# lucashilbig/BA_Pathtracing_Fur

Hardware: AMD Instinct MI355X
Metric: Msamples/s at 1080p 8spp, 1M-strand hairball; achieved HBM GB/s vs peak (higher is better)
Workload: dtype f32

## Files before the change

ba_pathtracing_fur_amd/csrc/render.hip:

```cpp
#include <hip/hip_runtime.h>
#include <rccl/rccl.h>
#include <stdio.h>
#include <string.h>

#include <algorithm>
#include <chrono>
#include <memory>
#include <string>
#include <condition_variable>
#include <deque>
#include <mutex>
#include <thread>
#include <type_traits>
#include <vector>

#include "device.h"
#include "device_build.h"
#include "lightpath.h"

using namespace khp;

#ifndef KHP_MAX_SEG
#define KHP_MAX_SEG 64
#endif
// ... 155 lines not shown
    c->nqb[0] = 0;
}

__global__ void k_prep(Counters* c, ShadowQ* q, int cur) {
    int nxt = cur ^ 1;
    c->nq[nxt] = 0;
    c->nqb[nxt] = 0;
    q->nsh = 0;
    q->nshb = 0;
    for (int g = 0; g < KHP_MAX_SEG; ++g) {
        c->fetch_ext[32 * g] = 0;
        q->fetch[32 * g] = 0;
    }
    c->ext_rays += c->nq[cur] + c->nqb[cur];
}

#ifndef KHP_EXT_RING
#define KHP_EXT_RING 8
#endif
#ifndef KHP_EXT_WAVES
#define KHP_EXT_WAVES 6
#endif
#ifndef KHP_EXT_REFILL
#define KHP_EXT_REFILL 24
#endif
#ifndef KHP_SH_RING
#define KHP_SH_RING 8
#endif
#ifndef KHP_SH_WAVES
#define KHP_SH_WAVES 6
#endif
constexpr int RING = KHP_SH_RING;
constexpr int REFILL = 24;
constexpr int TRAV_WAVES = KHP_SH_WAVES;
constexpr int EXT_RING = KHP_EXT_RING;
constexpr int EXT_WAVES = KHP_EXT_WAVES;
#ifndef KHP_EXT_WAVES_W
#define KHP_EXT_WAVES_W 6
#endif
constexpr int EXT_WAVES_W = KHP_EXT_WAVES_W;
#ifndef KHP_REFILL_CAM
#define KHP_REFILL_CAM 28
#endif
#ifndef KHP_REFILL_NARROW
#define KHP_REFILL_NARROW 28
#endif
#ifndef KHP_REFILL_WIDE
#define KHP_REFILL_WIDE 16
#endif
constexpr size_t LDS_BYTES = 3 * RING * TRAV_BLOCK * sizeof(uint32_t);
constexpr size_t EXT_LDS_BYTES = 3 * EXT_RING * TRAV_BLOCK * sizeof(uint32_t);
#ifndef KHP_CAM_RING
#define KHP_CAM_RING 6
#endif
#ifndef KHP_CAM_WAVES
#define KHP_CAM_WAVES 8
#endif
constexpr int CAM_RING = KHP_CAM_RING;
constexpr int CAM_WAVES = KHP_CAM_WAVES;
constexpr size_t CAM_LDS_BYTES = 3 * CAM_RING * TRAV_BLOCK * sizeof(uint32_t);
template <bool STATS, bool TOP = false>
using TravStack = LdsStack<RING, STATS, TOP>;
template <bool STATS, bool CAM = false, bool TOP = false>
using ExtStack = LdsStack<CAM ? CAM_RING : EXT_RING, STATS, TOP>;
constexpr size_t TOP_LDS_BYTES = TOP_NODES * sizeof(DevNode);

// ... 114 lines not shown
}

__device__ __forceinline__ void mark_pixel(const Wave& Wv, uint32_t pid, bool long_ray) {
    uint32_t fr, p_local, s_local;
    path_coords(Wv, pid, fr, p_local, s_local);
    Wv.pixheavy[Wv.pix[Wv.p_off + p_local]] = long_ray ? 1 : 0;
}

__global__ __launch_bounds__(256) void k_pix_order(const uint32_t* __restrict__ pix, uint32_t n,
                                                  const uint8_t* __restrict__ heavy, uint32_t* __restrict__ out,
                                                  uint32_t* cnt) {
    const uint32_t i = blockIdx.x * blockDim.x + threadIdx.x;
    const bool in = i < n;
    const uint32_t px = in ? pix[i] : 0u;
    const bool hv = in && heavy[px] != 0;
    const uint32_t f = wave_alloc(hv, &cnt[0]);
    const uint32_t b = wave_alloc(in && !hv, &cnt[1]);
    if (hv) out[f] = px;
    else if (in) out[n - 1u - b] = px;
}

template <bool STATS, bool CAM = false, bool WIDE = false, bool TOP = false>
__global__ __launch_bounds__(TRAV_BLOCK, WIDE ? EXT_WAVES_W : CAM ? CAM_WAVES : EXT_WAVES) void k_extend(DevScene S, Wave Wv, int cur, SpillArea spill) {
    extern __shared__ uint32_t lds[];
    const uint32_t nf = Wv.cnt->nq[cur], nb = Wv.cnt->nqb[cur];
    ExtStack<STATS, CAM, TOP> stk;
    stk.init(lds, spill.base, spill.stride);
    if (TOP) stk.stage_top(S.top);
    TravStats st{0, 0, 0};
    TravRay tr;
    Hit h;
    Cur c{0u, 0.0f, 0.0f, false};
    LeafCur lf{0u, 0u, 0.0f, 0.0f, 0.0f, 0.0f, -1};
    bool has = false, exhausted = false;
    uint32_t idx = 0, mode = 0u;
    unsigned long long wit = 0, wbusy = 0;
    uint32_t it = 0;
    Claimer cl;
    cl.init(Wv.cnt->fetch_ext, nf, nb, Wv.cap);
    constexpr int refill = WIDE ? KHP_REFILL_WIDE : CAM ? KHP_REFILL_CAM : KHP_REFILL_NARROW;
    for (;;) {
        unsigned long long idle = __ballot(!has);
        if (!exhausted && __popcll(idle) >= refill) {
            uint32_t my;
            const bool got = cl.claim(idle, my, exhausted);
            if (!has && got && cl.phys(my, idx)) {
                it = 0;
                Ray r;
                if (CAM) {
                    uint32_t key_unused;
                    r = camera_path(S, Wv, idx, key_unused);
                } else {
                    r.o = mk(Wv.qo[cur][0][idx], Wv.qo[cur][1][idx], Wv.qo[cur][2][idx]);
                    r.d = mk(Wv.qd[cur][0][idx], Wv.qd[cur][1][idx], Wv.qd[cur][2][idx]);
                }
                trav_setup(tr, r);
                h.t = FLT_MAX_;
                h.slot = -1;
                h.u = h.v = 0.0f;
                lf.left = 0;
                has = (STATS || !ray_has_nan(r)) && trav2_begin<STATS>(S, tr, h.t, stk, mode, c, lf, st);
                if (!has) {
                    Wv.ht[idx] = h.t;
                    Wv.hslot[idx] = -1;
                    Wv.heavy[idx] = 0;
                    if (CAM && Wv.pixheavy) mark_pixel(Wv, idx, false);
                }
            }
        }
        unsigned long long act = __ballot(has);
        if (act == 0) {
            if (exhausted) break;
            continue;
        }
        for (;;) {
            if (STATS) {
                unsigned long long wm = __ballot(has && (mode == M_NODE || mode == M_LEAF));
                ++wit;
                wbusy += (uint32_t)__popcll(wm);
            }
            if (has) {
                bool occ_unused;
                ++it;
                const bool fin = WIDE ? iterw<false, STATS>(S, tr, h, 0.0f, stk, mode, c, lf, st, occ_unused)
                                      : iter2<false, STATS>(S, tr, h, 0.0f, stk, mode, c, lf, st, occ_unused);
                if (fin) {
                    uint32_t j = idx;
                    asm volatile("" : "+v"(j));
                    Wv.ht[j] = h.t;
                    Wv.hslot[j] = h.slot;
                    Wv.heavy[j] = it > Wv.heavy_T ? 1 : 0;
                    if (CAM && Wv.pixheavy) mark_pixel(Wv, j, it > Wv.heavy_T);
                    has = false;
                }
            }
            act = __ballot(has);
            if (act == 0 || (!exhausted && 64 - __popcll(act) >= refill)) break;
        }
    }
    if (STATS)
        flush_stats(st, stk, wit, wbusy, &Wv.cnt->node_visits, &Wv.cnt->prim_tests, &Wv.cnt->pruned, &Wv.cnt->iters,
                    &Wv.cnt->lanes_busy, &Wv.cnt->spills);
}

static void launch_extend(bool stats, bool cam, bool wide, int grid, hipStream_t s, const DevScene& S, const Wave& W,
                          int cur, SpillArea sp, bool top = false) {
    const dim3 g(grid), b(TRAV_BLOCK);
    if (top && !stats && !wide && S.top) {
        if (cam) hipLaunchKernelGGL((k_extend<false, true, false, true>), g, b, CAM_LDS_BYTES + TOP_LDS_BYTES, s, S, W, cur, sp);
        else hipLaunchKernelGGL((k_extend<false, false, false, true>), g, b, EXT_LDS_BYTES + TOP_LDS_BYTES, s, S, W, cur, sp);
        return;
    }
#define KHP_EXT(ST, CA, WI) \
    hipLaunchKernelGGL((k_extend<ST, CA, WI>), g, b, CA ? CAM_LDS_BYTES : EXT_LDS_BYTES, s, S, W, cur, sp)
    if (wide) {
        if (stats) { if (cam) KHP_EXT(true, true, true); else KHP_EXT(true, false, true); }
        else { if (cam) KHP_EXT(false, true, true); else KHP_EXT(false, false, true); }
    } else {
        if (stats) { if (cam) KHP_EXT(true, true, false); else KHP_EXT(true, false, false); }
        else { if (cam) KHP_EXT(false, true, false); else KHP_EXT(false, false, false); }
    }
#undef KHP_EXT
}

__device__ __forceinline__ void textured_material(const DevScene& S, const Aux& ax, const float4* pr, v3 loc,
                                               const ShadeCtx& s, float bu, float bv, khp_material& out);
template <bool TEX>
__device__ __forceinline__ v3 surface_at(const DevScene& S, const Ray& r, const Hit& h, ShadeCtx& s,
                                         khp_material& mres) {
// ... 713 lines not shown
        const float4 f = rec[5];
        acc = acc + mk(f.x, f.y, f.z);
    }
    (void)pid;
    float4* dst = state_dest(Wv, nxt, bits_from_f(e.w));
    const float4 ck = *dst;
    *dst = make_float4(ck.x + acc.x, ck.y + acc.y, ck.z + acc.z, ck.w);
}

template <bool BD>
__global__ __launch_bounds__(256) void k_shadow_finish(DevScene S, Wave Wv, int nxt) {
    const uint32_t nf = Wv.shq->nsh, n = nf + Wv.shq->nshb;
    if (blockIdx.x == 0 && threadIdx.x == 0) atomicAdd(&Wv.cnt->sh_rays, (unsigned long long)n);
    for (uint32_t iv = blockIdx.x * blockDim.x + threadIdx.x; iv < n; iv += gridDim.x * blockDim.x) {
        const uint32_t i = q_phys(iv, nf, Wv.cap);
        if (BD) connection_group_finish(S, Wv, nxt, i);
        else shadow_finish_one(S, Wv, nxt, i, Wv.vis[i] != 0);
    }
}

template <bool STATS, bool WIDE = false, bool TOP = false>
__global__ __launch_bounds__(TRAV_BLOCK, TRAV_WAVES) void k_shadow(DevScene S, Wave Wv, SpillArea spill) {
    extern __shared__ uint32_t lds[];
    const uint32_t nf = Wv.shq->nsh, nb = Wv.shq->nshb;
    TravStack<STATS, TOP> stk;
    stk.init(lds, spill.base, spill.stride);
    if (TOP) stk.stage_top(S.top);
    TravStats st{0, 0, 0};
    TravRay tr;
    Cur c{0u, 0.0f, 0.0f, false};
    LeafCur lf{0u, 0u, 0.0f, 0.0f, 0.0f, 0.0f, -1};
    unsigned long long wit = 0, wbusy = 0;
    float tmax = 0.0f;
    uint32_t mode = 0u;
    bool has = false, exhausted = false;
    Claimer cl;
    cl.init(Wv.shq->fetch, nf, nb, Wv.cap);
    uint32_t idx = 0;
    for (;;) {
        unsigned long long idle = __ballot(!has);
        if (!exhausted && __popcll(idle) >= REFILL) {
            uint32_t my;
            const bool got = cl.claim(idle, my, exhausted);
            if (!has && got && cl.phys(my, idx)) {
                const float4* rec = Wv.sh + Wv.shs * (size_t)idx;
                float4 a = rec[0], b = rec[1];
                Ray r;
                r.o = mk(a.x, a.y, a.z);
                r.d = mk(b.x, b.y, b.z);
                tmax = a.w;
                trav_setup(tr, r);
                lf.left = 0;
                if (!STATS && x_slab_nan(tr)) {
                    has = false;
                    Wv.vis[idx] = any_hit_x_nan(S, r) ? 1 : 0;
                } else {
                    has = trav2_begin<STATS>(S, tr, tmax, stk, mode, c, lf, st);
                    if (!has) Wv.vis[idx] = 0;
                }
            }
        }
        unsigned long long act = __ballot(has);
        if (act == 0) {
            if (exhausted) break;
            continue;
        }
        for (;;) {
            if (STATS) {
                unsigned long long wm = __ballot(has && (mode == M_NODE || mode == M_LEAF));
                ++wit;
                wbusy += (uint32_t)__popcll(wm);
            }
            if (has) {
                bool occ = false;
                Hit hu_{0.0f, -1, 0.0f, 0.0f};
                const bool fin = WIDE ? iterw<true, STATS>(S, tr, hu_, tmax, stk, mode, c, lf, st, occ)
                                      : iter2<true, STATS>(S, tr, hu_, tmax, stk, mode, c, lf, st, occ);
                if (fin) {
                    Wv.vis[idx] = occ ? 1 : 0;
                    has = false;
                }
            }
            act = __ballot(has);
            if (act == 0 || (!exhausted && 64 - __popcll(act) >= REFILL)) break;
        }
    }
    if (STATS)
        flush_stats(st, stk, wit, wbusy, &Wv.cnt->sh_node_visits, &Wv.cnt->sh_prim_tests, &Wv.cnt->sh_pruned,
                    &Wv.cnt->sh_iters, &Wv.cnt->sh_lanes_busy, &Wv.cnt->spills);
}

static void launch_shadow(bool stats, bool wide, int grid, hipStream_t s, const DevScene& S, const Wave& W, SpillArea sp,
                          bool top = false) {
    const dim3 g(grid), b(TRAV_BLOCK);
    if (top && !stats && !wide && S.top) {
        hipLaunchKernelGGL((k_shadow<false, false, true>), g, b, LDS_BYTES + TOP_LDS_BYTES, s, S, W, sp);
        return;
    }
    if (wide) {
        if (stats) hipLaunchKernelGGL((k_shadow<true, true>), g, b, LDS_BYTES, s, S, W, sp);
        else hipLaunchKernelGGL((k_shadow<false, true>), g, b, LDS_BYTES, s, S, W, sp);
    } else {
        if (stats) hipLaunchKernelGGL((k_shadow<true, false>), g, b, LDS_BYTES, s, S, W, sp);
        else hipLaunchKernelGGL((k_shadow<false, false>), g, b, LDS_BYTES, s, S, W, sp);
    }
}

#ifndef KHP_PATH_WAVES
#define KHP_PATH_WAVES 4
#endif
#ifndef KHP_PATH_RING
#define KHP_PATH_RING 8
#endif
#ifndef KHP_PATH_REFILL
#define KHP_PATH_REFILL 24
#endif
// ... 3156 lines not shown
        Wv.shq->nsh = as_shadow ? n : 0u;
    }
    if (i >= n) return;
    Ray r = make_ray(ld3(orig + 3 * (size_t)i), ld3(dir + 3 * (size_t)i));
    if (as_shadow) {
        Wv.sh[Wv.shs * (size_t)i] = make_float4(r.o.x, r.o.y, r.o.z, tmax[i]);
        Wv.sh[Wv.shs * (size_t)i + 1] = make_float4(r.d.x, r.d.y, r.d.z, 0.0f);
    } else {
        Wv.qo[0][0][i] = r.o.x; Wv.qo[0][1][i] = r.o.y; Wv.qo[0][2][i] = r.o.z;
        Wv.qd[0][0][i] = r.d.x; Wv.qd[0][1][i] = r.d.y; Wv.qd[0][2][i] = r.d.z;
    }
}

__global__ void k_store_hits(DevScene S, uint32_t n, Wave Wv, float* t, int32_t* obj, float* uv) {
    uint32_t i = blockIdx.x * blockDim.x + threadIdx.x;
    if (i >= n) return;
    int32_t sl = Wv.hslot[i];
    t[i] = Wv.ht[i];
    obj[i] = sl >= 0 ? (int32_t)S.aux[sl].obj : -1;
    float u = 0.0f, v = 0.0f;
    if (sl >= 0) {
        const float4* p = S.prims + 4 * (size_t)sl;
        if (is_tri(p[0])) {
            Ray r;
            r.o = mk(Wv.qo[0][0][i], Wv.qo[0][1][i], Wv.qo[0][2][i]);
            r.d = mk(Wv.qd[0][0][i], Wv.qd[0][1][i], Wv.qd[0][2][i]);
            tri_uv(p[0], p[1], p[2], r, u, v);
        }
    }
    uv[2 * i] = u;
    uv[2 * i + 1] = v;
}

static int trace_persistent(const khp_ctx* c) { return (int)c->prm.trace_kernels; }

static khp_status trace_persistent_run(khp_ctx* c, uint32_t n, const float* orig, const float* dir,
                                       const float* tmax_h, float* t_out, int32_t* obj_out, float* uv_out,
                                       uint8_t* hit_out) {
    const bool shadow = hit_out != nullptr;
    PathSet& w = c->ps[0];
    c->wa.valid = false;
    khp_status s = ensure_wave(c, w, n);
    if (s != KHP_OK) return s;
    DevMem o, d, tm, t, ob, uv;
    HIPCHK(upload(o, orig, 3 * (size_t)n, c->stream));
    HIPCHK(upload(d, dir, 3 * (size_t)n, c->stream));
    if (shadow) HIPCHK(upload(tm, tmax_h, (size_t)n, c->stream));
    HIPCHK(hipMemsetAsync(w.cnt.p, 0, sizeof(Counters), c->stream));
    HIPCHK(hipMemsetAsync(w.shqb.p, 0, 2 * sizeof(ShadowQ), c->stream));
    Wave Wv = wave_view(c, w);
    hipLaunchKernelGGL(k_load_rays, dim3((n + 255) / 256), dim3(256), 0, c->stream, n, o.as<float>(), d.as<float>(),
                       Wv, shadow ? 1 : 0, tm.as<float>());
    const bool prod = trace_persistent(c) == 2;
    hipEvent_t e0 = next_event(c), e1 = next_event(c);
    (void)hipEventRecord(e0, c->stream);
    if (shadow) {
        SpillArea sp{w.spill_sh.as<int4>(), (uint32_t)c->grid_sh * TRAV_BLOCK};
        const bool wide = c->S.wide != nullptr && c->prm.wide_from == 0;
        launch_shadow(!prod, wide, wide ? c->grid_sh_w : c->grid_sh, c->stream, c->S, Wv, sp);
        (void)hipEventRecord(e1, c->stream);
        HIPCHK(hipGetLastError());
        HIPCHK(hipMemcpyAsync(hit_out, Wv.vis, n, hipMemcpyDeviceToHost, c->stream));
    } else {
        SpillArea sp{w.spill.as<int4>(), (uint32_t)c->grid_ext_max * TRAV_BLOCK};
        const bool wide = c->S.wide != nullptr && c->prm.wide_from == 0;
        launch_extend(!prod, false, wide, wide ? c->grid_ext_w : c->grid_ext, c->stream, c->S, Wv, 0, sp);
        (void)hipEventRecord(e1, c->stream);
        HIPCHK(t.ensure(4 * (size_t)n));
        HIPCHK(ob.ensure(4 * (size_t)n));
        HIPCHK(uv.ensure(8 * (size_t)n));
        hipLaunchKernelGGL(k_store_hits, dim3((n + 255) / 256), dim3(256), 0, c->stream, c->S, n, Wv, t.as<float>(),
                           ob.as<int32_t>(), uv.as<float>());
        HIPCHK(hipGetLastError());
        HIPCHK(hipMemcpyAsync(t_out, t.p, 4 * (size_t)n, hipMemcpyDeviceToHost, c->stream));
        HIPCHK(hipMemcpyAsync(obj_out, ob.p, 4 * (size_t)n, hipMemcpyDeviceToHost, c->stream));
        if (uv_out) HIPCHK(hipMemcpyAsync(uv_out, uv.p, 8 * (size_t)n, hipMemcpyDeviceToHost, c->stream));
    }
    Counters hc;
    HIPCHK(hipMemcpyAsync(&hc, w.cnt.p, sizeof(hc), hipMemcpyDeviceToHost, c->stream));
    KHPCHK(wait_stream(c, c->stream, "the ray queries"));
    c->st.node_visits = shadow ? hc.sh_node_visits : hc.node_visits;
    c->st.prim_tests = shadow ? hc.sh_prim_tests : hc.prim_tests;
    c->st.stack_spills = hc.spills;
    float kms = 0.0f;
    (void)hipEventElapsedTime(&kms, e0, e1);
    c->st.render_ms = kms;
    c->ev_next = 0;
    return KHP_OK;
}

extern "C" khp_status khp_trace_closest(khp_ctx* c, uint32_t n, const float* orig, const float* dir, float* t_out,
                                        int32_t* obj_out, float* uv_out) {
    if (c) {
        khp_status dr = drain(c);
        if (dr != KHP_OK) return dr;
    }
    if (!c || (n && (!orig || !dir || !t_out || !obj_out))) return fail(KHP_EINVAL, "null argument");
    if (!c->built) return fail(KHP_ENOTREADY, "khp_build_accel first");
    if (n == 0) return KHP_OK;
    HIPCHK(hipSetDevice(c->device));
    if (trace_persistent(c)) return trace_persistent_run(c, n, orig, dir, nullptr, t_out, obj_out, uv_out, nullptr);
    DevMem o, d, t, ob, uv, stb;
    HIPCHK(upload(o, orig, 3 * (size_t)n, c->stream));
    HIPCHK(upload(d, dir, 3 * (size_t)n, c->stream));
    HIPCHK(t.ensure(4 * (size_t)n));
    HIPCHK(ob.ensure(4 * (size_t)n));
    HIPCHK(uv.ensure(8 * (size_t)n));
    HIPCHK(stb.ensure(16));
    HIPCHK(hipMemsetAsync(stb.p, 0, 16, c->stream));
    hipLaunchKernelGGL(k_trace_closest<true>, dim3((n + 255) / 256), dim3(256), 0, c->stream, c->S, n,
                       o.as<float>(), d.as<float>(), t.as<float>(), ob.as<int32_t>(), uv.as<float>(),
                       stb.as<unsigned long long>());
    HIPCHK(hipGetLastError());
    HIPCHK(hipMemcpyAsync(t_out, t.p, 4 * (size_t)n, hipMemcpyDeviceToHost, c->stream));
    HIPCHK(hipMemcpyAsync(obj_out, ob.p, 4 * (size_t)n, hipMemcpyDeviceToHost, c->stream));
    if (uv_out) HIPCHK(hipMemcpyAsync(uv_out, uv.p, 8 * (size_t)n, hipMemcpyDeviceToHost, c->stream));
// ... 443 lines not shown
```

ba_pathtracing_fur_amd/csrc/traverse.h:

```cpp
#pragma once

struct Hit {
    float t;
    int32_t slot;
    float u, v;
};

struct TravStats {
    uint32_t nodes, prims, pruned;
};

struct TravRay {
    Ray r;
    v3 inv;
    bool fin;
};

__device__ __forceinline__ void trav_setup(TravRay& tr, const Ray& r) {
    tr.r = r;
    tr.inv = mk(1.0f / r.d.x, 1.0f / r.d.y, 1.0f / r.d.z);
    tr.fin = __builtin_isfinite(tr.inv.x) && __builtin_isfinite(tr.inv.y) && __builtin_isfinite(tr.inv.z) &&
             __builtin_isfinite(r.o.x) && __builtin_isfinite(r.o.y) && __builtin_isfinite(r.o.z);
}

__device__ __forceinline__ bool ray_has_nan(const Ray& r) {
    return r.o.x != r.o.x || r.o.y != r.o.y || r.o.z != r.o.z || r.d.x != r.d.x || r.d.y != r.d.y ||
           r.d.z != r.d.z;
}

__device__ __forceinline__ bool x_slab_nan(const TravRay& tr) { return tr.inv.x != tr.inv.x || tr.r.o.x != tr.r.o.x; }
__device__ __forceinline__ bool any_hit_x_nan(const DevScene& S, const Ray& r) {
    for (uint32_t k = 0; k < S.n_tris; ++k) {
        const float4* p = S.prims + 4 * (size_t)S.tri_slot[k];
        const float4 ab = p[1], ac = p[2];
        const v3 dv = cross(r.d, mk(ac.x, ac.y, ac.z));
        const float det = dot(dv, mk(ab.x, ab.y, ab.z));
        if (!(fabsf(det) < TRI_EPS_D)) return true;
    }
    return false;
}

__device__ __forceinline__ bool ref_leaf(uint32_t r) { return (r & LEAF_BIT) != 0u; }

struct PrivStack {
    uint32_t ref[STACK_MAX];
    float t0[STACK_MAX], t1[STACK_MAX];
    int sp;
    __device__ __forceinline__ void clear() { sp = 0; }
    __device__ __forceinline__ bool empty() const { return sp == 0; }
    __device__ __forceinline__ void push(uint32_t r, float a, float b) {
        ref[sp] = r;
        t0[sp] = a;
        t1[sp] = b;
        ++sp;
    }
    __device__ __forceinline__ void pop(uint32_t& r, float& a, float& b) {
        --sp;
        r = ref[sp];
        a = t0[sp];
        b = t1[sp];
    }
};

#ifndef KHP_TRAV_BLOCK
#define KHP_TRAV_BLOCK 64
#endif
constexpr uint32_t TRAV_BLOCK = KHP_TRAV_BLOCK;

constexpr uint32_t TOP_NODES = 7;
constexpr uint32_t TOP_REF = 0x40000000u;
template <int R, bool COUNT, bool TOP = false>
struct LdsStack {
    static_assert(R >= 2 && R <= 16, "ring size");
    static constexpr bool kTop = TOP;
    static constexpr size_t kRingBytes = 3 * (size_t)R * TRAV_BLOCK * sizeof(uint32_t);
// ... 21 lines not shown
    __device__ __forceinline__ bool empty() const { return sp == 0; }
    __device__ __forceinline__ uint32_t slot(int e) const { return (uint32_t)((uint32_t)e % (uint32_t)R) * TRAV_BLOCK + threadIdx.x; }
    __device__ __forceinline__ int4* gcell(int e) const {
        return spill + (size_t)e * stride + blockIdx.x * blockDim.x + threadIdx.x;
    }
    __device__ __forceinline__ void push(uint32_t r, float a, float b) {
        if (sp - lo == R) {
            uint32_t k = slot(lo);
            *gcell(lo) = make_int4((int)lds[k], (int)lds[k + R * TRAV_BLOCK], (int)lds[k + 2 * R * TRAV_BLOCK], 0);
            ++lo;
            if (COUNT) ++spills;
        }
        uint32_t k = slot(sp);
        lds[k] = r;
        lds[k + R * TRAV_BLOCK] = bits_from_f(a);
        lds[k + 2 * R * TRAV_BLOCK] = bits_from_f(b);
        ++sp;
    }
    __device__ __forceinline__ void pop(uint32_t& r, float& a, float& b) {
        --sp;
        const uint32_t k = slot(sp);
        r = lds[k];
        a = f_from_bits(lds[k + R * TRAV_BLOCK]);
        b = f_from_bits(lds[k + 2 * R * TRAV_BLOCK]);
        asm volatile("" : "+v"(r), "+v"(a), "+v"(b));
        if (sp < lo) {
            int4 e = *gcell(sp);
            r = (uint32_t)e.x;
            a = f_from_bits((uint32_t)e.y);
            b = f_from_bits((uint32_t)e.z);
            lo = sp;
        }
    }
};

__device__ __forceinline__ void pin(float4& v) { asm volatile("" : "+v"(v.x), "+v"(v.y), "+v"(v.z), "+v"(v.w)); }
__device__ __forceinline__ void pin(int4& v) { asm volatile("" : "+v"(v.x), "+v"(v.y), "+v"(v.z), "+v"(v.w)); }

struct Cur {
    uint32_t ref;
    float t0, t1;
    bool valid;
};

template <class Stack>
__device__ __forceinline__ void cur_next(Stack& stk, Cur& c) {
    if (stk.empty()) {
        c.valid = false;
    } else {
        stk.pop(c.ref, c.t0, c.t1);
        c.valid = true;
    }
}


template <class Stack>
__device__ __forceinline__ bool trav_begin(const DevScene& S, const TravRay& tr, Stack& stk, Cur& c) {
    stk.clear();
    float t0, t1;
    c.valid = slab(S.root_box[0], S.root_box[1], S.root_box[2], S.root_box[3], S.root_box[4], S.root_box[5], tr.r,
                   tr.inv, t0, t1);
    c.ref = (uint32_t)S.root_ref;
    c.t0 = t0;
    c.t1 = t1;
    return c.valid;
}
// ... 152 lines not shown
    t0 = (tzmin > tmin) ? tzmin : tmin;
    t1 = (tzmax < tmax) ? tzmax : tmax;
    return ok;
}

__device__ __forceinline__ bool slab_fast(float mnx, float mny, float mnz, float mxx, float mxy, float mxz,
                                          const TravRay& tr, float& t0, float& t1) {
    const float ax = (mnx - tr.r.o.x) * tr.inv.x, bx = (mxx - tr.r.o.x) * tr.inv.x;
    const float ay = (mny - tr.r.o.y) * tr.inv.y, by = (mxy - tr.r.o.y) * tr.inv.y;
    const float az = (mnz - tr.r.o.z) * tr.inv.z, bz = (mxz - tr.r.o.z) * tr.inv.z;
    t0 = fmaxf(fmaxf(fminf(ax, bx), fminf(ay, by)), fminf(az, bz));
    t1 = fminf(fminf(fmaxf(ax, bx), fmaxf(ay, by)), fmaxf(az, bz));
    return t0 <= t1;
}

template <bool STATS>
__device__ __forceinline__ void take_entry(const DevScene& S, uint32_t ref, float t0, float t1, uint32_t& mode, Cur& c,
                                           LeafCur& lf, TravStats& st) {
    const bool leaf = ref_leaf(ref);
    c.ref = ref;
    c.t0 = t0;
    c.t1 = t1;
    mode = leaf ? M_LEAF : M_NODE;
    uint32_t cnt = (ref >> 24) & 0x7Fu;
    if (leaf && cnt == LEAF_CNT_ESC) cnt = S.aux[ref & 0x00FFFFFFu].flags >> 8;
    lf.slot = leaf ? (ref & 0x00FFFFFFu) : lf.slot;
    lf.left = leaf ? cnt : 0u;
    lf.tmax = t1;
    lf.tl = FLT_MAX_;
    lf.lu = 0.0f;
    lf.lv = 0.0f;
    lf.sl = -1;
    if (STATS && leaf) st.nodes++;
}

template <bool STATS, class Stack>
__device__ __forceinline__ bool trav2_begin(const DevScene& S, const TravRay& tr, float tlimit, Stack& stk,
                                            uint32_t& mode, Cur& c, LeafCur& lf, TravStats& st) {
    stk.clear();
    float t0, t1;
    if (!slab(S.root_box[0], S.root_box[1], S.root_box[2], S.root_box[3], S.root_box[4], S.root_box[5], tr.r,
              tr.inv, t0, t1))
        return false;
    if (t1 < 0.0f || t0 > tlimit) {
        if (STATS) st.pruned++;
        mode = M_POP;
        return true;
    }
    take_entry<STATS>(S, (uint32_t)(Stack::kTop ? S.top_root : S.root_ref), t0, t1, mode, c, lf, st);
    return true;
}

__device__ __forceinline__ bool candidate_rt(float4 p0, float4 p1, float4 p2, float4 p3, const Ray& r, bool any,
                                             float tMax, float& t) {
    if (is_tri(p0)) {
        float u, v;
        return tri_test(p0, p1, p2, r, 0.0f, tMax, t, u, v);
    }
    return cone_quadratic(p0, p1, p2, p3, r, any, 0.0f, tMax, t);
}

#ifdef KHP_LEAF_REUSE
__device__ unsigned long long g_leaf_hist[16 * 8];
__device__ uint32_t g_reuse_b;
__device__ __forceinline__ void leaf_reuse(bool in_leaf, uint32_t slot) {
    unsigned long long m = __ballot(in_leaf);
// ... 10 lines not shown
            atomicAdd(&g_leaf_hist[b * 8 + 7], 1ull);
        }
        m &= ~same;
    }
}
#endif

template <int KIND, bool STATS, class Stack>
__device__ __forceinline__ bool iter2k(const DevScene& S, const TravRay& tr, Hit& h, float tmax_any, Stack& stk,
                                       uint32_t& mode, Cur& c, LeafCur& lf, TravStats& st, bool& occluded,
                                       bool any_rt) {
    const bool ANY = KIND == 2 ? any_rt : KIND == 1;
    const bool in_leaf = mode == M_LEAF;
    const bool fetch = in_leaf || mode == M_NODE;
    const float4* p = in_leaf ? S.prims + 4 * (size_t)lf.slot : reinterpret_cast<const float4*>(S.nodes + c.ref);
#ifdef KHP_LEAF_REUSE
    if (STATS && KIND == 0) leaf_reuse(in_leaf, lf.slot);
#endif
    float4 q0, q1, q2, q3;
    if (Stack::kTop && fetch && !in_leaf && (c.ref & TOP_REF) != 0u) {
        const float4* t = stk.top() + 4 * (c.ref & 0xFFu);
        q0 = t[0];
        q1 = t[1];
        q2 = t[2];
        q3 = t[3];
    } else if (fetch) {
        q0 = p[0];
        q1 = p[1];
        q2 = p[2];
        q3 = p[3];
        pin(q0); pin(q1); pin(q2); pin(q3);
    }
    bool need_pop = mode == M_POP;
    bool have = false;
    uint32_t eref = 0u;
    float et0 = 0.0f, et1 = 0.0f;
    bool push = false;
    uint32_t pref = 0u;
    float pt0 = 0.0f, pt1 = 0.0f;
    if (in_leaf) {
        if (STATS) st.prims++;
        if (KIND == 2) {
            float t = 0.0f;
            const bool ok = candidate_rt(q0, q1, q2, q3, tr.r, ANY, ANY ? tmax_any : lf.tmax, t);
            if (ok && ANY) {
                occluded = true;
                return true;
            }
            if (ok) {
                lf.sl = (int32_t)lf.slot;
                lf.tmax = t;
            }
        } else if (ANY) {
            if (any_candidate(q0, q1, q2, q3, tr.r, tmax_any)) {
                occluded = true;
                return true;
            }
        } else {
            leaf_candidate_t(q0, q1, q2, q3, (int32_t)lf.slot, tr.r, lf.tmax, lf.sl);
        }
        ++lf.slot;
        --lf.left;
        if (lf.left == 0u) {
            if (!ANY && lf.sl >= 0 && lf.tmax < h.t) {
                h.t = lf.tmax;
                h.slot = lf.sl;
            }
            need_pop = true;
        }
    } else if (fetch) {
        if (STATS) st.nodes++;
        const float tlimit = ANY ? tmax_any : h.t;
        float l0, l1, r0, r1;
        bool lh, rh;
        if (__ballot(!tr.fin) == 0ull) {
            lh = slab_fast(q0.x, q0.y, q0.z, q0.w, q1.x, q1.y, tr, l0, l1);
            rh = slab_fast(q1.z, q1.w, q2.x, q2.y, q2.z, q2.w, tr, r0, r1);
        } else {
            lh = slab_sel(q0.x, q0.y, q0.z, q0.w, q1.x, q1.y, tr, l0, l1);
            rh = slab_sel(q1.z, q1.w, q2.x, q2.y, q2.z, q2.w, tr, r0, r1);
        }
        lh = lh && !(l1 < 0.0f || l0 > tlimit);
        rh = rh && !(r1 < 0.0f || r0 > tlimit);
        const uint32_t lref = __float_as_uint(q3.x), rref = __float_as_uint(q3.y);
        const bool nearl = lh && (!rh || l0 < r0);
        have = lh || rh;
        need_pop = !have;
        push = lh && rh;
        eref = nearl ? lref : rref;
        et0 = nearl ? l0 : r0;
        et1 = nearl ? l1 : r1;
        pref = nearl ? rref : lref;
        pt0 = nearl ? r0 : l0;
        pt1 = nearl ? r1 : l1;
    }
    if (push) stk.push(pref, pt0, pt1);
    if (need_pop) {
        if (stk.empty()) {
            mode = M_IDLE;
            occluded = false;
            return true;
        }
        stk.pop(eref, et0, et1);
        const float tlimit = ANY ? tmax_any : h.t;
        if (et1 < 0.0f || et0 > tlimit) {
            if (STATS) st.pruned++;
            mode = M_POP;
        } else {
            have = true;
        }
    }
    if (have) take_entry<STATS>(S, eref, et0, et1, mode, c, lf, st);
    return false;
}

template <bool ANY, bool STATS, class Stack>
__device__ __forceinline__ bool iter2(const DevScene& S, const TravRay& tr, Hit& h, float tmax_any, Stack& stk,
                                      uint32_t& mode, Cur& c, LeafCur& lf, TravStats& st, bool& occluded) {
    return iter2k<ANY ? 1 : 0, STATS>(S, tr, h, tmax_any, stk, mode, c, lf, st, occluded, ANY);
}

struct WBox {
    float e0, e1, e2, x0, x1, x2;
};
__device__ __forceinline__ WBox wbox_fast(float mnx, float mny, float mnz, float mxx, float mxy, float mxz,
                                          const TravRay& tr) {
    const float ax = (mnx - tr.r.o.x) * tr.inv.x, bx = (mxx - tr.r.o.x) * tr.inv.x;
    const float ay = (mny - tr.r.o.y) * tr.inv.y, by = (mxy - tr.r.o.y) * tr.inv.y;
    const float az = (mnz - tr.r.o.z) * tr.inv.z, bz = (mxz - tr.r.o.z) * tr.inv.z;
    return WBox{fminf(ax, bx), fminf(ay, by), fminf(az, bz), fmaxf(ax, bx), fmaxf(ay, by), fmaxf(az, bz)};
}
__device__ __forceinline__ WBox wbox_union(const WBox& a, const WBox& b) {
    return WBox{fminf(a.e0, b.e0), fminf(a.e1, b.e1), fminf(a.e2, b.e2),
                fmaxf(a.x0, b.x0), fmaxf(a.x1, b.x1), fmaxf(a.x2, b.x2)};
}
__device__ __forceinline__ bool wbox_t(const WBox& w, float& t0, float& t1) {
    t0 = fmaxf(fmaxf(w.e0, w.e1), w.e2);
    t1 = fminf(fminf(w.x0, w.x1), w.x2);
    return t0 <= t1;
}
__device__ __forceinline__ float wmin(float a, float b) { return (b < a) ? b : a; }
__device__ __forceinline__ float wmax(float a, float b) { return (a < b) ? b : a; }

template <int KIND, bool STATS, class Stack>
__device__ __forceinline__ bool iterwk(const DevScene& S, const TravRay& tr, Hit& h, float tmax_any, Stack& stk,
                                       uint32_t& mode, Cur& c, LeafCur& lf, TravStats& st, bool& occluded,
                                       bool any_rt) {
    const bool ANY = KIND == 2 ? any_rt : KIND == 1;
    if (__ballot(!tr.fin) != 0ull)
        return iter2k<KIND, STATS>(S, tr, h, tmax_any, stk, mode, c, lf, st, occluded, any_rt);
    const bool in_leaf = mode == M_LEAF;
    const bool node = mode == M_NODE;
    const bool fetch = in_leaf || node;
    const float4* p = in_leaf ? S.prims + 4 * (size_t)lf.slot : S.wide + 8 * (size_t)c.ref;
#ifdef KHP_LEAF_REUSE
    if (STATS && KIND == 0) leaf_reuse(in_leaf, lf.slot);
#endif
    float4 q0, q1, q2, q3, q4, q5, q6, q7;
    if (fetch) {
        q0 = p[0];
        q1 = p[1];
        q2 = p[2];
        q3 = p[3];
    }
    if (node) {
        q4 = p[4];
        q5 = p[5];
        q6 = p[6];
        q7 = p[7];
    }
    if (fetch) {
        pin(q0); pin(q1); pin(q2); pin(q3);
    }
    if (node) {
        pin(q4); pin(q5); pin(q6); pin(q7);
    }
    bool need_pop = mode == M_POP;
    bool have = false;
    uint32_t eref = 0u;
    float et0 = 0.0f, et1 = 0.0f;
    bool push1 = false, push2 = false;
    uint32_t p1ref = 0u, p2ref = 0u;
    float p1t0 = 0.0f, p1t1 = 0.0f, p2t0 = 0.0f, p2t1 = 0.0f;
    if (in_leaf) {
        if (STATS) st.prims++;
        if (KIND == 2) {
            float t = 0.0f;
            const bool ok = candidate_rt(q0, q1, q2, q3, tr.r, ANY, ANY ? tmax_any : lf.tmax, t);
            if (ok && ANY) {
                occluded = true;
                return true;
            }
            if (ok) {
                lf.sl = (int32_t)lf.slot;
                lf.tmax = t;
            }
        } else if (ANY) {
            if (any_candidate(q0, q1, q2, q3, tr.r, tmax_any)) {
                occluded = true;
                return true;
            }
        } else {
            leaf_candidate_t(q0, q1, q2, q3, (int32_t)lf.slot, tr.r, lf.tmax, lf.sl);
        }
        ++lf.slot;
        --lf.left;
        if (lf.left == 0u) {
            if (!ANY && lf.sl >= 0 && lf.tmax < h.t) {
                h.t = lf.tmax;
                h.slot = lf.sl;
            }
            need_pop = true;
        }
    } else if (node) {
        if (STATS) st.nodes++;
        const float tlimit = ANY ? tmax_any : h.t;
        const uint32_t c1 = __float_as_uint(q6.x), c2 = __float_as_uint(q6.y);
        const bool i1 = !ref_leaf(c1), i2 = !ref_leaf(c2);
        float gt0[4], gt1[4], At0, At1, Bt0, Bt1;
        bool gh[4], hA, hB;
        {
            const WBox w0 = wbox_fast(q0.x, q0.y, q0.z, q0.w, q1.x, q1.y, tr);
            const WBox w1 = wbox_fast(q1.z, q1.w, q2.x, q2.y, q2.z, q2.w, tr);
            const WBox w2 = wbox_fast(q3.x, q3.y, q3.z, q3.w, q4.x, q4.y, tr);
            const WBox w3 = wbox_fast(q4.z, q4.w, q5.x, q5.y, q5.z, q5.w, tr);
            gh[0] = wbox_t(w0, gt0[0], gt1[0]);
            gh[1] = wbox_t(w1, gt0[1], gt1[1]);
            gh[2] = wbox_t(w2, gt0[2], gt1[2]);
            gh[3] = wbox_t(w3, gt0[3], gt1[3]);
            const WBox wa = wbox_union(w0, w1), wb = wbox_union(w2, w3);
            float ua0, ua1, ub0, ub1;
            const bool ua = wbox_t(wa, ua0, ua1), ub = wbox_t(wb, ub0, ub1);
            hA = i1 ? ua : gh[0];
            At0 = i1 ? ua0 : gt0[0];
// ... 5 lines not shown
        hA = hA && !(At1 < 0.0f || At0 > tlimit);
        hB = hB && !(Bt1 < 0.0f || Bt0 > tlimit);
        const bool nearA = hA && (!hB || At0 < Bt0);
        const bool have_near = hA || hB;
        const uint32_t nref = nearA ? c1 : c2;
        const bool nint = have_near && !ref_leaf(nref);
        const bool fhit = hA && hB;
        const uint32_t fref = nearA ? c2 : c1;
        const float f0 = nearA ? Bt0 : At0, f1 = nearA ? Bt1 : At1;
        const uint32_t glref = __float_as_uint(nearA ? q6.z : q7.x), grref = __float_as_uint(nearA ? q6.w : q7.y);
        const float gl0 = nearA ? gt0[0] : gt0[2], gl1 = nearA ? gt1[0] : gt1[2];
        const float gr0 = nearA ? gt0[1] : gt0[3], gr1 = nearA ? gt1[1] : gt1[3];
        const bool hl = nint && (nearA ? gh[0] : gh[2]) && !(gl1 < 0.0f || gl0 > tlimit);
        const bool hr = nint && (nearA ? gh[1] : gh[3]) && !(gr1 < 0.0f || gr0 > tlimit);
        const bool gnl = hl && (!hr || gl0 < gr0);
        const bool have_g = hl || hr;
        if (STATS && nint) st.nodes++;
        const uint32_t gref = gnl ? glref : grref;
        const float g0 = gnl ? gl0 : gr0, g1 = gnl ? gl1 : gr1;
        eref = !nint ? nref : (have_g ? gref : fref);
        et0 = !nint ? (nearA ? At0 : Bt0) : (have_g ? g0 : f0);
        et1 = !nint ? (nearA ? At1 : Bt1) : (have_g ? g1 : f1);
        have = have_near && (!nint || have_g || fhit);
        need_pop = !have;
        push1 = fhit && (!nint || have_g);
        p1ref = fref;
        p1t0 = f0;
        p1t1 = f1;
        push2 = hl && hr;
        p2ref = gnl ? grref : glref;
        p2t0 = gnl ? gr0 : gl0;
        p2t1 = gnl ? gr1 : gl1;
    }
    if (push1) stk.push(p1ref, p1t0, p1t1);
    if (push2) stk.push(p2ref, p2t0, p2t1);
    if (need_pop) {
        if (stk.empty()) {
            mode = M_IDLE;
            occluded = false;
            return true;
        }
        stk.pop(eref, et0, et1);
        if (et1 < 0.0f || et0 > (ANY ? tmax_any : h.t)) {
            if (STATS) st.pruned++;
            mode = M_POP;
        } else {
            have = true;
        }
    }
    if (have) take_entry<STATS>(S, eref, et0, et1, mode, c, lf, st);
    return false;
}

template <bool ANY, bool STATS, class Stack>
__device__ __forceinline__ bool iterw(const DevScene& S, const TravRay& tr, Hit& h, float tmax_any, Stack& stk,
                                      uint32_t& mode, Cur& c, LeafCur& lf, TravStats& st, bool& occluded) {
    return iterwk<ANY ? 1 : 0, STATS>(S, tr, h, tmax_any, stk, mode, c, lf, st, occluded, ANY);
}

template <bool STATS, class Stack>
__device__ __forceinline__ void trace_closest(const DevScene& S, const Ray& r, Hit& h, Stack& stk, TravStats& st) {
    h.t = FLT_MAX_;
    h.slot = -1;
    h.u = h.v = 0.0f;
    TravRay tr;
    trav_setup(tr, r);
    Cur c;
    if (!trav_begin(S, tr, stk, c)) return;
    while (c.valid) {
        if (ref_leaf(c.ref)) leaf_step_closest<STATS>(S, tr, h, stk, c, st);
        else interior_step<STATS>(S, tr, h.t, stk, c, st);
    }
}

template <bool STATS, class Stack>
__device__ __forceinline__ bool trace_any(const DevScene& S, const Ray& r, float tMaxRay, Stack& stk, TravStats& st) {
    TravRay tr;
    trav_setup(tr, r);
    Cur c;
    if (!trav_begin(S, tr, stk, c)) return false;
    while (c.valid) {
        if (ref_leaf(c.ref)) {
            if (leaf_step_any<STATS>(S, tr, tMaxRay, stk, c, st)) return true;
        } else {
// ... 6 lines not shown
```

Measured before the change: 692.8.

## Make traversal step branchless with predicated stack ops and deferred result writes

Replaces early returns and divergent push/pop branches in the BVH iteration with predicated push_sel/pop_sel and a select-based stack_step, so every lane runs the same instruction stream each step. The persistent extend and shadow kernels now track lane activity through mode rather than a separate has flag, and write each ray's result at the top of the next loop pass instead of inside the divergent finish branch. The goal is to cut wave divergence and reconvergence overhead in the hot traversal loop. In exchange, idle lanes still perform the LDS reads of a pop, and a sentinel-check validation kernel plus extra memsets are added to the persistent query path.

```diff
diff --git a/ba_pathtracing_fur_amd/csrc/render.hip b/ba_pathtracing_fur_amd/csrc/render.hip
--- a/ba_pathtracing_fur_amd/csrc/render.hip
+++ b/ba_pathtracing_fur_amd/csrc/render.hip
@@ -211,6 +211,7 @@
 #endif
 constexpr int RING = KHP_SH_RING;
 constexpr int REFILL = 24;
+constexpr uint32_t NO_SLOT = 0xFFFFFFFFu;
 constexpr int TRAV_WAVES = KHP_SH_WAVES;
 constexpr int EXT_RING = KHP_EXT_RING;
 constexpr int EXT_WAVES = KHP_EXT_WAVES;
@@ -391,19 +392,32 @@
     Hit h;
     Cur c{0u, 0.0f, 0.0f, false};
     LeafCur lf{0u, 0u, 0.0f, 0.0f, 0.0f, 0.0f, -1};
-    bool has = false, exhausted = false;
-    uint32_t idx = 0, mode = 0u;
+    tr.fin = true;
+    bool exhausted = false;
+    uint32_t idx = NO_SLOT, mode = M_IDLE;
     unsigned long long wit = 0, wbusy = 0;
     uint32_t it = 0;
     Claimer cl;
     cl.init(Wv.cnt->fetch_ext, nf, nb, Wv.cap);
     constexpr int refill = WIDE ? KHP_REFILL_WIDE : CAM ? KHP_REFILL_CAM : KHP_REFILL_NARROW;
+    unsigned long long act = 0ull;
     for (;;) {
-        unsigned long long idle = __ballot(!has);
-        if (!exhausted && __popcll(idle) >= refill) {
-            uint32_t my;
-            const bool got = cl.claim(idle, my, exhausted);
-            if (!has && got && cl.phys(my, idx)) {
+        if (idx != NO_SLOT && mode == M_IDLE) {
+            Wv.ht[idx] = h.t;
+            Wv.hslot[idx] = h.slot;
+            Wv.heavy[idx] = it > Wv.heavy_T ? 1 : 0;
+            if (CAM && Wv.pixheavy) mark_pixel(Wv, idx, it > Wv.heavy_T);
+            idx = NO_SLOT;
+        }
+        if (exhausted && act == 0) break;
+        if (!exhausted && 64 - __popcll(act) >= refill) {
+            uint32_t my, slot;
+            const bool has = mode != M_IDLE;
+            bool done = false;
+            const bool got = cl.claim(~act, my, done);
+            exhausted = __builtin_amdgcn_readfirstlane(done ? 1 : 0) != 0;
+            if (!has && got && cl.phys(my, slot)) {
+                idx = slot;
                 it = 0;
                 Ray r;
                 if (CAM) {
@@ -418,42 +432,23 @@
                 h.slot = -1;
                 h.u = h.v = 0.0f;
                 lf.left = 0;
-                has = (STATS || !ray_has_nan(r)) && trav2_begin<STATS>(S, tr, h.t, stk, mode, c, lf, st);
-                if (!has) {
-                    Wv.ht[idx] = h.t;
-                    Wv.hslot[idx] = -1;
-                    Wv.heavy[idx] = 0;
-                    if (CAM && Wv.pixheavy) mark_pixel(Wv, idx, false);
-                }
-            }
-        }
-        unsigned long long act = __ballot(has);
-        if (act == 0) {
-            if (exhausted) break;
-            continue;
-        }
+                const bool go = (STATS || !ray_has_nan(r)) && trav2_begin<STATS>(S, tr, h.t, stk, mode, c, lf, st);
+                if (!go) mode = M_IDLE;
+            }
+        }
+        act = wave_ballot(mode != M_IDLE);
+        if (act == 0) continue;
         for (;;) {
             if (STATS) {
-                unsigned long long wm = __ballot(has && (mode == M_NODE || mode == M_LEAF));
+                unsigned long long wm = wave_ballot(mode == M_NODE || mode == M_LEAF);
                 ++wit;
                 wbusy += (uint32_t)__popcll(wm);
             }
-            if (has) {
-                bool occ_unused;
-                ++it;
-                const bool fin = WIDE ? iterw<false, STATS>(S, tr, h, 0.0f, stk, mode, c, lf, st, occ_unused)
-                                      : iter2<false, STATS>(S, tr, h, 0.0f, stk, mode, c, lf, st, occ_unused);
-                if (fin) {
-                    uint32_t j = idx;
-                    asm volatile("" : "+v"(j));
-                    Wv.ht[j] = h.t;
-                    Wv.hslot[j] = h.slot;
-                    Wv.heavy[j] = it > Wv.heavy_T ? 1 : 0;
-                    if (CAM && Wv.pixheavy) mark_pixel(Wv, j, it > Wv.heavy_T);
-                    has = false;
-                }
-            }
-            act = __ballot(has);
+            bool occ_unused = false;
+            it += mode != M_IDLE ? 1u : 0u;
+            if (WIDE) iterw<false, STATS>(S, tr, h, 0.0f, stk, mode, c, lf, st, occ_unused);
+            else iter2<false, STATS>(S, tr, h, 0.0f, stk, mode, c, lf, st, occ_unused);
+            act = wave_ballot(mode != M_IDLE);
             if (act == 0 || (!exhausted && 64 - __popcll(act) >= refill)) break;
         }
     }
@@ -1233,17 +1228,28 @@
     LeafCur lf{0u, 0u, 0.0f, 0.0f, 0.0f, 0.0f, -1};
     unsigned long long wit = 0, wbusy = 0;
     float tmax = 0.0f;
-    uint32_t mode = 0u;
-    bool has = false, exhausted = false;
+    tr.fin = true;
+    uint32_t mode = M_IDLE;
+    bool exhausted = false, occ = false;
     Claimer cl;
     cl.init(Wv.shq->fetch, nf, nb, Wv.cap);
-    uint32_t idx = 0;
+    uint32_t idx = NO_SLOT;
+    unsigned long long act = 0ull;
     for (;;) {
-        unsigned long long idle = __ballot(!has);
-        if (!exhausted && __popcll(idle) >= REFILL) {
-            uint32_t my;
-            const bool got = cl.claim(idle, my, exhausted);
-            if (!has && got && cl.phys(my, idx)) {
+        if (idx != NO_SLOT && mode == M_IDLE) {
+            Wv.vis[idx] = occ ? 1 : 0;
+            idx = NO_SLOT;
+        }
+        if (exhausted && act == 0) break;
+        if (!exhausted && 64 - __popcll(act) >= REFILL) {
+            uint32_t my, slot;
+            const bool has = mode != M_IDLE;
+            bool done = false;
+            const bool got = cl.claim(~act, my, done);
+            exhausted = __builtin_amdgcn_readfirstlane(done ? 1 : 0) != 0;
+            if (!has && got && cl.phys(my, slot)) {
+                idx = slot;
+                occ = false;
                 const float4* rec = Wv.sh + Wv.shs * (size_t)idx;
                 float4 a = rec[0], b = rec[1];
                 Ray r;
@@ -1252,37 +1258,28 @@
                 tmax = a.w;
                 trav_setup(tr, r);
                 lf.left = 0;
+                bool go;
                 if (!STATS && x_slab_nan(tr)) {
-                    has = false;
-                    Wv.vis[idx] = any_hit_x_nan(S, r) ? 1 : 0;
+                    go = false;
+                    occ = any_hit_x_nan(S, r);
                 } else {
-                    has = trav2_begin<STATS>(S, tr, tmax, stk, mode, c, lf, st);
-                    if (!has) Wv.vis[idx] = 0;
+                    go = trav2_begin<STATS>(S, tr, tmax, stk, mode, c, lf, st);
                 }
-            }
-        }
-        unsigned long long act = __ballot(has);
-        if (act == 0) {
-            if (exhausted) break;
-            continue;
-        }
+                if (!go) mode = M_IDLE;
+            }
+        }
+        act = wave_ballot(mode != M_IDLE);
+        if (act == 0) continue;
         for (;;) {
             if (STATS) {
-                unsigned long long wm = __ballot(has && (mode == M_NODE || mode == M_LEAF));
+                unsigned long long wm = wave_ballot(mode == M_NODE || mode == M_LEAF);
                 ++wit;
                 wbusy += (uint32_t)__popcll(wm);
             }
-            if (has) {
-                bool occ = false;
-                Hit hu_{0.0f, -1, 0.0f, 0.0f};
-                const bool fin = WIDE ? iterw<true, STATS>(S, tr, hu_, tmax, stk, mode, c, lf, st, occ)
-                                      : iter2<true, STATS>(S, tr, hu_, tmax, stk, mode, c, lf, st, occ);
-                if (fin) {
-                    Wv.vis[idx] = occ ? 1 : 0;
-                    has = false;
-                }
-            }
-            act = __ballot(has);
+            Hit hu_{0.0f, -1, 0.0f, 0.0f};
+            if (WIDE) iterw<true, STATS>(S, tr, hu_, tmax, stk, mode, c, lf, st, occ);
+            else iter2<true, STATS>(S, tr, hu_, tmax, stk, mode, c, lf, st, occ);
+            act = wave_ballot(mode != M_IDLE);
             if (act == 0 || (!exhausted && 64 - __popcll(act) >= REFILL)) break;
         }
     }
@@ -4505,6 +4502,17 @@
     uv[2 * i + 1] = v;
 }
 
+constexpr int TRACE_SENTINEL = 0xEE;
+__global__ void k_check_sentinel(uint32_t n, uint32_t cap, const uint32_t* ht, const uint32_t* hslot, const uint8_t* vis,
+                                 int as_shadow, uint32_t* bad) {
+    const uint32_t i = blockIdx.x * blockDim.x + threadIdx.x;
+    if (i >= cap) return;
+    const uint32_t w = 0x01010101u * (uint32_t)TRACE_SENTINEL;
+    const bool left = as_shadow ? vis[i] == (uint8_t)TRACE_SENTINEL : (ht[i] == w || hslot[i] == w);
+    const bool touched = as_shadow ? vis[i] != (uint8_t)TRACE_SENTINEL : (ht[i] != w || hslot[i] != w);
+    if (i < n ? left : touched) atomicAdd(&bad[i < n ? 0 : 1], 1u);
+}
+
 static int trace_persistent(const khp_ctx* c) { return (int)c->prm.trace_kernels; }
 
 static khp_status trace_persistent_run(khp_ctx* c, uint32_t n, const float* orig, const float* dir,
@@ -4522,6 +4530,15 @@
     HIPCHK(hipMemsetAsync(w.cnt.p, 0, sizeof(Counters), c->stream));
     HIPCHK(hipMemsetAsync(w.shqb.p, 0, 2 * sizeof(ShadowQ), c->stream));
     Wave Wv = wave_view(c, w);
+    DevMem bad;
+    HIPCHK(bad.ensure(2 * sizeof(uint32_t)));
+    HIPCHK(hipMemsetAsync(bad.p, 0, 2 * sizeof(uint32_t), c->stream));
+    if (shadow) {
+        HIPCHK(hipMemsetAsync(Wv.vis, TRACE_SENTINEL, w.cap, c->stream));
+    } else {
+        HIPCHK(hipMemsetAsync(Wv.ht, TRACE_SENTINEL, w.cap * 4, c->stream));
+        HIPCHK(hipMemsetAsync(Wv.hslot, TRACE_SENTINEL, w.cap * 4, c->stream));
+    }
     hipLaunchKernelGGL(k_load_rays, dim3((n + 255) / 256), dim3(256), 0, c->stream, n, o.as<float>(), d.as<float>(),
                        Wv, shadow ? 1 : 0, tm.as<float>());
     const bool prod = trace_persistent(c) == 2;
@@ -4549,12 +4566,25 @@
         HIPCHK(hipMemcpyAsync(obj_out, ob.p, 4 * (size_t)n, hipMemcpyDeviceToHost, c->stream));
         if (uv_out) HIPCHK(hipMemcpyAsync(uv_out, uv.p, 8 * (size_t)n, hipMemcpyDeviceToHost, c->stream));
     }
+    const uint32_t cap = (uint32_t)w.cap;
+    hipLaunchKernelGGL(k_check_sentinel, dim3((cap + 255) / 256), dim3(256), 0, c->stream, n, cap,
+                       reinterpret_cast<const uint32_t*>(Wv.ht), reinterpret_cast<const uint32_t*>(Wv.hslot), Wv.vis,
+                       shadow ? 1 : 0, bad.as<uint32_t>());
+    HIPCHK(hipGetLastError());
+    uint32_t hbad[2] = {0u, 0u};
+    HIPCHK(hipMemcpyAsync(hbad, bad.p, sizeof(hbad), hipMemcpyDeviceToHost, c->stream));
     Counters hc;
     HIPCHK(hipMemcpyAsync(&hc, w.cnt.p, sizeof(hc), hipMemcpyDeviceToHost, c->stream));
     KHPCHK(wait_stream(c, c->stream, "the ray queries"));
+    if (hbad[0] || hbad[1])
+        return fail(KHP_EDEVICE, "persistent query: " + std::to_string(hbad[0]) + " of " + std::to_string(n) +
+                                     " results never written, " + std::to_string(hbad[1]) +
+                                     " slots past the queue written");
     c->st.node_visits = shadow ? hc.sh_node_visits : hc.node_visits;
     c->st.prim_tests = shadow ? hc.sh_prim_tests : hc.prim_tests;
     c->st.stack_spills = hc.spills;
+    if (shadow) c->st.shadow_pruned_pops = hc.sh_pruned;
+    else c->st.extend_pruned_pops = hc.pruned;
     float kms = 0.0f;
     (void)hipEventElapsedTime(&kms, e0, e1);
     c->st.render_ms = kms;
diff --git a/ba_pathtracing_fur_amd/csrc/traverse.h b/ba_pathtracing_fur_amd/csrc/traverse.h
--- a/ba_pathtracing_fur_amd/csrc/traverse.h
+++ b/ba_pathtracing_fur_amd/csrc/traverse.h
@@ -41,6 +41,8 @@
 }
 
 __device__ __forceinline__ bool ref_leaf(uint32_t r) { return (r & LEAF_BIT) != 0u; }
+
+__device__ __forceinline__ unsigned long long wave_ballot(bool p) { return __builtin_amdgcn_ballot_w64(p); }
 
 struct PrivStack {
     uint32_t ref[STACK_MAX];
@@ -128,6 +130,37 @@
             lo = sp;
         }
     }
+    __device__ __forceinline__ void push_sel(bool on, uint32_t r, float a, float b) {
+        if (on && sp - lo == R) {
+            uint32_t k = slot(lo);
+            *gcell(lo) = make_int4((int)lds[k], (int)lds[k + R * TRAV_BLOCK], (int)lds[k + 2 * R * TRAV_BLOCK], 0);
+            ++lo;
+            if (COUNT) ++spills;
+        }
+        if (on) {
+            uint32_t k = slot(sp);
+            lds[k] = r;
+            lds[k + R * TRAV_BLOCK] = bits_from_f(a);
+            lds[k + 2 * R * TRAV_BLOCK] = bits_from_f(b);
+        }
+        sp += on ? 1 : 0;
+    }
+    __device__ __forceinline__ void pop_sel(bool want, uint32_t& r, float& a, float& b) {
+        const int top = sp - 1;
+        const uint32_t k = slot(top);
+        r = lds[k];
+        a = f_from_bits(lds[k + R * TRAV_BLOCK]);
+        b = f_from_bits(lds[k + 2 * R * TRAV_BLOCK]);
+        asm volatile("" : "+v"(r), "+v"(a), "+v"(b));
+        if (want && top < lo) {
+            int4 e = *gcell(top);
+            r = (uint32_t)e.x;
+            a = f_from_bits((uint32_t)e.y);
+            b = f_from_bits((uint32_t)e.z);
+            lo = top;
+        }
+        sp = want ? top : sp;
+    }
 };
 
 __device__ __forceinline__ void pin(float4& v) { asm volatile("" : "+v"(v.x), "+v"(v.y), "+v"(v.z), "+v"(v.w)); }
@@ -346,6 +379,43 @@
     lf.lv = 0.0f;
     lf.sl = -1;
     if (STATS && leaf) st.nodes++;
+}
+
+template <bool STATS, class Stack>
+__device__ __forceinline__ bool stack_step(const DevScene& S, Stack& stk, float tlimit, bool occ, bool need_pop,
+                                           bool have, uint32_t eref, float et0, float et1, uint32_t& mode, Cur& c,
+                                           LeafCur& lf, TravStats& st) {
+    need_pop = need_pop && !occ;
+    const bool empty = stk.empty();
+    const bool want = need_pop && !empty;
+    const bool fin = occ || (need_pop && empty);
+    uint32_t pr;
+    float p0, p1;
+    stk.pop_sel(want, pr, p0, p1);
+    const bool pruned = want && (p1 < 0.0f || p0 > tlimit);
+    if (STATS) st.pruned += pruned ? 1u : 0u;
+    const bool take = have || (want && !pruned);
+    eref = have ? eref : pr;
+    et0 = have ? et0 : p0;
+    et1 = have ? et1 : p1;
+    const bool leaf = take && ref_leaf(eref);
+    uint32_t cnt = (eref >> 24) & 0x7Fu;
+    if (leaf && cnt == LEAF_CNT_ESC) cnt = S.aux[eref & 0x00FFFFFFu].flags >> 8;
+    c.ref = take ? eref : c.ref;
+    c.t0 = take ? et0 : c.t0;
+    c.t1 = take ? et1 : c.t1;
+    mode = take ? (leaf ? M_LEAF : M_NODE) : mode;
+    mode = pruned ? M_POP : mode;
+    mode = fin ? M_IDLE : mode;
+    lf.slot = leaf ? (eref & 0x00FFFFFFu) : lf.slot;
+    lf.left = take ? (leaf ? cnt : 0u) : lf.left;
+    lf.tmax = take ? et1 : lf.tmax;
+    lf.tl = take ? FLT_MAX_ : lf.tl;
+    lf.lu = take ? 0.0f : lf.lu;
+    lf.lv = take ? 0.0f : lf.lv;
+    lf.sl = take ? -1 : lf.sl;
+    if (STATS) st.nodes += leaf ? 1u : 0u;
+    return fin;
 }
 
 template <bool STATS, class Stack>
@@ -422,6 +492,7 @@
         pin(q0); pin(q1); pin(q2); pin(q3);
     }
     bool need_pop = mode == M_POP;
+    bool occ = false;
     bool have = false;
     uint32_t eref = 0u;
     float et0 = 0.0f, et1 = 0.0f;
@@ -433,19 +504,13 @@
         if (KIND == 2) {
             float t = 0.0f;
             const bool ok = candidate_rt(q0, q1, q2, q3, tr.r, ANY, ANY ? tmax_any : lf.tmax, t);
-            if (ok && ANY) {
-                occluded = true;
-                return true;
-            }
+            occ = ok && ANY;
             if (ok) {
                 lf.sl = (int32_t)lf.slot;
                 lf.tmax = t;
             }
         } else if (ANY) {
-            if (any_candidate(q0, q1, q2, q3, tr.r, tmax_any)) {
-                occluded = true;
-                return true;
-            }
+            occ = any_candidate(q0, q1, q2, q3, tr.r, tmax_any);
         } else {
             leaf_candidate_t(q0, q1, q2, q3, (int32_t)lf.slot, tr.r, lf.tmax, lf.sl);
         }
@@ -484,24 +549,9 @@
         pt0 = nearl ? r0 : l0;
         pt1 = nearl ? r1 : l1;
     }
-    if (push) stk.push(pref, pt0, pt1);
-    if (need_pop) {
-        if (stk.empty()) {
-            mode = M_IDLE;
-            occluded = false;
-            return true;
-        }
-        stk.pop(eref, et0, et1);
-        const float tlimit = ANY ? tmax_any : h.t;
-        if (et1 < 0.0f || et0 > tlimit) {
-            if (STATS) st.pruned++;
-            mode = M_POP;
-        } else {
-            have = true;
-        }
-    }
-    if (have) take_entry<STATS>(S, eref, et0, et1, mode, c, lf, st);
-    return false;
+    stk.push_sel(push, pref, pt0, pt1);
+    if (KIND != 0) occluded = occluded || occ;
+    return stack_step<STATS>(S, stk, ANY ? tmax_any : h.t, occ, need_pop, have, eref, et0, et1, mode, c, lf, st);
 }
 
 template <bool ANY, bool STATS, class Stack>
@@ -566,6 +616,7 @@
         pin(q4); pin(q5); pin(q6); pin(q7);
     }
     bool need_pop = mode == M_POP;
+    bool occ = false;
     bool have = false;
     uint32_t eref = 0u;
     float et0 = 0.0f, et1 = 0.0f;
@@ -577,19 +628,13 @@
         if (KIND == 2) {
             float t = 0.0f;
             const bool ok = candidate_rt(q0, q1, q2, q3, tr.r, ANY, ANY ? tmax_any : lf.tmax, t);
-            if (ok && ANY) {
-                occluded = true;
-                return true;
-            }
+            occ = ok && ANY;
             if (ok) {
                 lf.sl = (int32_t)lf.slot;
                 lf.tmax = t;
             }
         } else if (ANY) {
-            if (any_candidate(q0, q1, q2, q3, tr.r, tmax_any)) {
-                occluded = true;
-                return true;
-            }
+            occ = any_candidate(q0, q1, q2, q3, tr.r, tmax_any);
         } else {
             leaf_candidate_t(q0, q1, q2, q3, (int32_t)lf.slot, tr.r, lf.tmax, lf.sl);
         }
@@ -661,24 +706,10 @@
         p2t0 = gnl ? gr0 : gl0;
         p2t1 = gnl ? gr1 : gl1;
     }
-    if (push1) stk.push(p1ref, p1t0, p1t1);
-    if (push2) stk.push(p2ref, p2t0, p2t1);
-    if (need_pop) {
-        if (stk.empty()) {
-            mode = M_IDLE;
-            occluded = false;
-            return true;
-        }
-        stk.pop(eref, et0, et1);
-        if (et1 < 0.0f || et0 > (ANY ? tmax_any : h.t)) {
-            if (STATS) st.pruned++;
-            mode = M_POP;
-        } else {
-            have = true;
-        }
-    }
-    if (have) take_entry<STATS>(S, eref, et0, et1, mode, c, lf, st);
-    return false;
+    stk.push_sel(push1, p1ref, p1t0, p1t1);
+    stk.push_sel(push2, p2ref, p2t0, p2t1);
+    if (KIND != 0) occluded = occluded || occ;
+    return stack_step<STATS>(S, stk, ANY ? tmax_any : h.t, occ, need_pop, have, eref, et0, et1, mode, c, lf, st);
 }
 
 template <bool ANY, bool STATS, class Stack>
```

After: 713.4, median of 6. 3.0% higher.
